# kostas1515/object_detectors

Measured on AMD Instinct MI355X. Metric: images/sec (fwd+bwd) YOLOv3 640px bs=32, higher is better.
Workload: dtype bf16; 1 GPU; YOLOv3 Darknet-53 training step (fwd+loss+bwd+SGD step), synthetic COCO 640px, per-GPU bs=32, 7 GT/img, random-init weights; global_batch=32, parallelism=dp1

## Files before the change

object_detectors_amd/csrc/wgrad_kernels.hip:

```cpp
#include "common.h"

#include <cstdlib>
#include <unordered_map>

#include "tune_record.h"

using namespace mi355;

typedef __attribute__((ext_vector_type(4))) short s16x4_t;
typedef __attribute__((ext_vector_type(4))) float f32x4_t;

struct FastDiv {
  unsigned mul, shift, d;
};

static FastDiv make_fastdiv(unsigned d) {
  FastDiv f;
  f.d = d;
  unsigned l = 0;
  while ((1ull << l) < d) ++l;
  f.shift = l;
  f.mul = (unsigned)(((1ull << 32) * ((1ull << l) - d)) / d + 1);
  return f;
}
__device__ __forceinline__ unsigned fdiv(unsigned n, const FastDiv f) {
  const unsigned t = __umulhi(f.mul, n);
  return (t + n) >> f.shift;
}

struct WgradParams {
  const bf16_t* x;
  const bf16_t* dy;
  float* dw;
  float* slab;
  const bf16_t* zero;
  int M, Ho, Wo, H, W, ldx, lddy, Cin, Cout, stride, pad, ks, T, NP;
  int co_tiles, np_tiles, splits, chunk;
  int step_q, step_r;
  FastDiv dWo, dHo, dCin;
  int ablate;
};

int g_wgrad_ablate = 0;
int g_wgrad_general = 0;
int g_conv_strict = 0;
int g_wgrad_force_dbg = 0;
int g_wgrad8_off = 0;

namespace {

#define WG_BKP 64
#define WG_TILE 128
#define WG_ROWB 256

__device__ __forceinline__ void glds16(const void* gsrc, void* lds_dst_uniform) {
  __builtin_amdgcn_global_load_lds((const __attribute__((address_space(1))) void*)gsrc,
                                   (__attribute__((address_space(3))) void*)lds_dst_uniform, 16, 0, 0);
}

typedef __attribute__((ext_vector_type(4))) int srd_t;
__device__ __forceinline__ srd_t make_srd(const void* base, unsigned num_records) {
  const unsigned long long a = (unsigned long long)base;
  srd_t r;
  r[0] = (int)(unsigned)a;
  r[1] = (int)((unsigned)(a >> 32) & 0xFFFFu);
  r[2] = (int)num_records;
  r[3] = 0x00020000;
  return r;
}
__device__ __forceinline__ void bufld16(srd_t rsrc, const void* lds_dst_uniform, int voffset, int soffset) {
  const unsigned lds = (unsigned)(unsigned long long)(__attribute__((address_space(3))) const void*)lds_dst_uniform;
  asm volatile("s_mov_b32 m0, %0\n\ts_nop 0\n\tbuffer_load_dwordx4 %1, %2, %3 offen lds" ::"s"(lds), "v"(voffset), "s"(rsrc), "s"(soffset) : "memory");
}
#define OOB_VOFF ((int)0x80000000)

__device__ __forceinline__ int rowf(int row) { return (row & 3) | (((row >> 3) & 1) << 2); }

__device__ __forceinline__ st16x4_t lds_tr(const char* p) {
  s16x4_t v = __builtin_amdgcn_ds_read_tr16_b64_v4i16((__attribute__((address_space(3))) s16x4_t*)p);
  return __builtin_bit_cast(st16x4_t, v);
}

template <int CI, int CJ, int GRP4>
__global__ __launch_bounds__(256, 2) void wgrad_kernel(const WgradParams p) {
  constexpr int STAGE = 2 * WG_BKP * WG_ROWB;
  extern __shared__ __attribute__((aligned(16))) char smem[];
  const int tid = threadIdx.x, lane = tid & 63;
  const int wid = __builtin_amdgcn_readfirstlane(tid >> 6);
  const int wr = wid & 1, wc = wid >> 1;

  int bid = blockIdx.x;
  {
    const int nblk = gridDim.x, q = nblk / 8, r = nblk % 8, xcd = bid % 8, loc = bid / 8;
    bid = (xcd < r ? xcd * (q + 1) : r * (q + 1) + (xcd - r) * q) + loc;
  }
  const int tiles = p.co_tiles * p.np_tiles;
  const int split = bid / tiles, tile = bid - split * tiles;
  const int ct = tile % p.co_tiles, nt = tile / p.co_tiles;
  const int co0 = ct * WG_TILE, np0 = nt * WG_TILE;
  const int mA = split * p.chunk, mB = min(p.M, mA + p.chunk);
  if (mA >= mB) return;

  const int lrow = lane >> 4, cpos = lane & 15;
  int x_off[2], x_tapdy[2], x_tapdx[2], dy_off[2];
  bool x_ok[2];
#pragma unroll
  for (int ph = 0; ph < 2; ++ph) {
    const int f = (lrow & 3) | (ph << 2);
    const int gchunk = (((cpos >> 1) ^ f) << 1) | (cpos & 1);
    dy_off[ph] = co0 + gchunk * 8;
    const int np = np0 + gchunk * 8;
    x_ok[ph] = np < p.NP;
    const int t = x_ok[ph] ? (int)fdiv((unsigned)np, p.dCin) : 0;
    const int ci = np - t * p.Cin;
    const int kh = t / p.ks, kw = t - kh * p.ks;
    x_tapdy[ph] = kh - p.pad;
    x_tapdx[ph] = kw - p.pad;
    x_off[ph] = ci;
  }
  const bool dy_ok0 = dy_off[0] < p.Cout, dy_ok1 = dy_off[1] < p.Cout;

  int r_n[4], r_ho[4], r_wo[4];
#pragma unroll
  for (int i = 0; i < 4; ++i) {
    if (GRP4) break;
    const unsigned um = (unsigned)(mA + (wid * 4 + i) * 4 + lrow);
    const unsigned q1 = fdiv(um, p.dWo);
    r_wo[i] = (int)(um - q1 * p.Wo);
    const unsigned n = fdiv(q1, p.dHo);
    r_ho[i] = (int)(q1 - n * p.Ho);
    r_n[i] = (int)n;
  }

  int g_hs[4], g_ws[4], g_sb[4], dyv[4], lc[2], ty[2], cx[2];
  srd_t rsrc_x;
  const int WoS = p.Wo * p.stride, HoS = p.Ho * p.stride;
  const int c_ws = p.step_r * p.stride, c_hs = p.step_q * p.stride;
  const int c_sb = (c_hs * p.W + c_ws) * p.ldx * 2;
  const int c_row = (p.stride * p.W - WoS) * p.ldx * 2;
  const int c_img = (p.H - HoS) * p.W * p.ldx * 2;
  const int c_piece = 4 * p.stride * p.ldx * 2;
  if constexpr (GRP4 != 0) {
#pragma unroll
    for (int i = 0; i < 4; ++i) {
      const unsigned um = (unsigned)(mA + (wid * 4 + i) * 4);
      const unsigned q1 = fdiv(um, p.dWo);
      const int wo = (int)(um - q1 * p.Wo);
      const unsigned n = fdiv(q1, p.dHo);
      const int ho = (int)(q1 - n * p.Ho);
      g_hs[i] = ho * p.stride;
      g_ws[i] = wo * p.stride;
      g_sb[i] = (((int)n * p.H + g_hs[i]) * p.W + g_ws[i]) * p.ldx * 2;
      const int ph = (i >> 1) & 1;
      dyv[i] = (ph ? dy_ok1 : dy_ok0) ? (((wid * 4 + i) * 4 + lrow) * p.lddy + dy_off[ph]) * 2 : OOB_VOFF;
    }
#pragma unroll
    for (int ph = 0; ph < 2; ++ph) {
      lc[ph] = (((x_tapdy[ph] + p.pad) * p.W + lrow * p.stride + x_tapdx[ph] + p.pad) * p.ldx + x_off[ph]) * 2;
      ty[ph] = x_ok[ph] ? x_tapdy[ph] : -(1 << 24);
      cx[ph] = lrow * p.stride + x_tapdx[ph];
    }
    rsrc_x = make_srd(p.x - (p.pad * p.W + p.pad) * p.ldx, 0x7FFFFFF0u);
  }
  auto stage_grp4 = [&](int m_base, int buf) {
    char* sd = smem + buf * STAGE;
    char* sx = sd + WG_BKP * WG_ROWB;
    const int rem = mB - m_base;
    const srd_t rsrc_dy = make_srd(p.dy + (long long)m_base * p.lddy, (unsigned)(rem * p.lddy * 2));
#pragma unroll
    for (int i = 0; i < 4; ++i) {
      const int instr = wid * 4 + i;
      const int ph = (i >> 1) & 1;
      if (!(p.ablate & 2) || m_base == mA) bufld16(rsrc_dy, sd + instr * 1024, dyv[i], 0);
      if (GRP4 == 3) {
        const int hs = g_hs[0], ws = g_ws[0] + i * 4 * p.stride;
        const bool ok = instr * 4 < rem && (unsigned)(hs + ty[ph]) < (unsigned)p.H && (unsigned)(ws + cx[ph]) < (unsigned)p.W;
        if (!(p.ablate & 1) || m_base == mA) bufld16(rsrc_x, sx + instr * 1024, ok ? lc[ph] : OOB_VOFF, g_sb[0] + i * c_piece);
        if (i < 3) continue;
      }
      const int ti = GRP4 == 3 ? 0 : i;
      const int hs = g_hs[ti], ws = g_ws[ti];
      if (GRP4 == 3) {
      } else if (GRP4 == 1 || (ws + 4 * p.stride <= WoS && instr * 4 + 4 <= rem)) {
        const bool ok = instr * 4 < rem && (unsigned)(hs + ty[ph]) < (unsigned)p.H && (unsigned)(ws + cx[ph]) < (unsigned)p.W;
        if (!(p.ablate & 1) || m_base == mA) bufld16(rsrc_x, sx + instr * 1024, ok ? lc[ph] : OOB_VOFF, g_sb[i]);
      } else {
        const bool last_row = hs + p.stride == HoS;
        const int hs1 = last_row ? 0 : hs + p.stride;
        const int ex1 = c_row + (last_row ? c_img : 0);
        const bool wr = ws + lrow * p.stride >= WoS;
        const int iy = (wr ? hs1 : hs) + ty[ph];
        const int ix = ws + cx[ph] - (wr ? WoS : 0);
        const bool ok = instr * 4 + lrow < rem && (unsigned)iy < (unsigned)p.H && (unsigned)ix < (unsigned)p.W;
        bufld16(rsrc_x, sx + instr * 1024, ok ? lc[ph] + (wr ? ex1 : 0) : OOB_VOFF, g_sb[i]);
      }
      g_ws[ti] += c_ws;
      g_hs[ti] += c_hs;
      g_sb[ti] += c_sb;
      if (g_ws[ti] >= WoS) {
        g_ws[ti] -= WoS;
        g_hs[ti] += p.stride;
        g_sb[ti] += c_row;
      }
      if (g_hs[ti] >= HoS) {
        g_hs[ti] -= HoS;
        g_sb[ti] += c_img;
      }
    }
  };

  auto stage_any = [&](int m_base, int buf) {
    char* sd = smem + buf * STAGE;
    char* sx = sd + WG_BKP * WG_ROWB;
#pragma unroll
    for (int i = 0; i < 4; ++i) {
      const int instr = wid * 4 + i;
      const int row = instr * 4 + lrow;
      const int ph = (row >> 3) & 1;
      const int m = m_base + row;
      const bool mv = m < mB;
      const bf16_t* sdy = (mv && (ph ? dy_ok1 : dy_ok0)) ? p.dy + (long long)m * p.lddy + (ph ? dy_off[1] : dy_off[0]) : p.zero;
      glds16(sdy, sd + instr * 1024);
      const int iy = r_ho[i] * p.stride + (ph ? x_tapdy[1] : x_tapdy[0]);
      const int ix = r_wo[i] * p.stride + (ph ? x_tapdx[1] : x_tapdx[0]);
      const bool ok = mv && (ph ? x_ok[1] : x_ok[0]) && iy >= 0 && iy < p.H && ix >= 0 && ix < p.W;
      const bf16_t* sxp = ok ? p.x + ((long long)(r_n[i] * p.H + iy) * p.W + ix) * p.ldx + (ph ? x_off[1] : x_off[0]) : p.zero;
      glds16(sxp, sx + instr * 1024);
      r_wo[i] += p.step_r;
      r_ho[i] += p.step_q;
      if (r_wo[i] >= p.Wo) {
        r_wo[i] -= p.Wo;
        r_ho[i] += 1;
      }
      while (r_ho[i] >= p.Ho) {
        r_ho[i] -= p.Ho;
        r_n[i] += 1;
      }
    }
  };

  auto stage = [&](int m_base, int buf) {
    if constexpr (GRP4 != 0)
      stage_grp4(m_base, buf);
    else
      stage_any(m_base, buf);
  };

  f32x4_t acc[CI][CJ];
#pragma unroll
  for (int i = 0; i < CI; ++i)
#pragma unroll
    for (int j = 0; j < CJ; ++j) acc[i][j] = {0.f, 0.f, 0.f, 0.f};

  const int ksteps = (mB - mA + WG_BKP - 1) / WG_BKP;
  stage(mA, 0);
  asm volatile("s_waitcnt vmcnt(0)" ::: "memory");
  __syncthreads();

  const int g = lane >> 4, q = (lane & 15) >> 2, pp = lane & 3;
  for (int s = 0; s < ksteps; ++s) {
    const int buf = s & 1;
    if (s + 1 < ksteps) stage(mA + (s + 1) * WG_BKP, buf ^ 1);
    const char* sd = smem + buf * STAGE;
    const char* sx = sd + WG_BKP * WG_ROWB;
#pragma unroll
    for (int ks = 0; ks < WG_BKP / 32; ++ks) {
      st16x8_t af[CI], bfr[CJ];
#pragma unroll
      for (int h = 0; h < 2; ++h) {
        const int row = ks * 32 + 8 * g + 4 * h + q;
        const int f = rowf(row);
#pragma unroll
        for (int i = 0; i < CI; ++i) {
          const int blk = wr * CI + i;
          const st16x4_t v = lds_tr(sd + row * WG_ROWB + ((blk ^ f) << 5) + pp * 8);
          af[i][4 * h + 0] = v[0];
          af[i][4 * h + 1] = v[1];
          af[i][4 * h + 2] = v[2];
          af[i][4 * h + 3] = v[3];
        }
#pragma unroll
        for (int j = 0; j < CJ; ++j) {
          const int blk = wc * CJ + j;
          const st16x4_t v = lds_tr(sx + row * WG_ROWB + ((blk ^ f) << 5) + pp * 8);
          bfr[j][4 * h + 0] = v[0];
          bfr[j][4 * h + 1] = v[1];
          bfr[j][4 * h + 2] = v[2];
          bfr[j][4 * h + 3] = v[3];
        }
      }
      if (!(p.ablate & 4)) {
#pragma unroll
        for (int i = 0; i < CI; ++i)
#pragma unroll
          for (int j = 0; j < CJ; ++j) acc[i][j] = MI355_MFMA_16x16x32(af[i], bfr[j], acc[i][j]);
      } else {
        acc[0][0][0] += (float)af[0][0] + (float)bfr[0][0];
      }
    }
    asm volatile("s_waitcnt vmcnt(0)" ::: "memory");
    __syncthreads();
  }

  const int fr = lane & 15, fq = lane >> 4;
  if (p.slab) {
    float* dst = p.slab + ((size_t)split * tiles + tile) * (WG_TILE * WG_TILE);
#pragma unroll
    for (int i = 0; i < CI; ++i)
#pragma unroll
      for (int r = 0; r < 4; ++r)
#pragma unroll
        for (int j = 0; j < CJ; ++j)
          dst[((wr * CI + i) * 16 + fq * 4 + r) * WG_TILE + (wc * CJ + j) * 16 + fr] = acc[i][j][r];
    return;
  }
#pragma unroll
  for (int i = 0; i < CI; ++i) {
#pragma unroll
    for (int r = 0; r < 4; ++r) {
      const int co = co0 + (wr * CI + i) * 16 + fq * 4 + r;
      if (co >= p.Cout) continue;
#pragma unroll
      for (int j = 0; j < CJ; ++j) {
        const int np = np0 + (wc * CJ + j) * 16 + fr;
        if (np < p.NP) p.dw[(long long)co * p.NP + np] += acc[i][j][r];
      }
    }
  }
}

constexpr int W8_HALF = WG_BKP * WG_ROWB;
constexpr int W8_STAGE = 4 * W8_HALF;
constexpr int W8_LDS = 2 * W8_STAGE;
constexpr int W8_TILE = 256;

template <int N>
__device__ __forceinline__ void w8_wait_vm() {
  asm volatile("s_waitcnt vmcnt(%0)" ::"n"(N) : "memory");
}
__device__ __forceinline__ void w8_bar() {
  asm volatile("" ::: "memory");
  __builtin_amdgcn_s_barrier();
  asm volatile("" ::: "memory");
}

template <bool STRADDLE>
__global__ __launch_bounds__(512, 2) void wgrad8_kernel(const WgradParams p) {
  extern __shared__ __attribute__((aligned(16))) char smem[];
  const int tid = threadIdx.x, lane = tid & 63;
  const int wid = __builtin_amdgcn_readfirstlane(tid >> 6);
  const int wm = wid >> 2, wn = wid & 3;

  int bid = blockIdx.x;
  {
    const int nblk = gridDim.x, q = nblk / 8, r = nblk % 8, xcd = bid % 8, loc = bid / 8;
    bid = (xcd < r ? xcd * (q + 1) : r * (q + 1) + (xcd - r) * q) + loc;
  }
  const int co_tiles8 = (p.Cout + W8_TILE - 1) / W8_TILE, np_tiles8 = (p.NP + W8_TILE - 1) / W8_TILE;
  const int tiles8 = co_tiles8 * np_tiles8;
  const int split = bid / tiles8, tile = bid - split * tiles8;
  const int CT = tile % co_tiles8, NT = tile / co_tiles8;
  const int co0 = CT * W8_TILE, np0 = NT * W8_TILE;
  const int mA = split * p.chunk, mB = min(p.M, mA + p.chunk);
  if (mA >= mB) return;
  const int mlen = mB - mA;

  const int lrow = lane >> 4, cpos = lane & 15;
  const int fst = lrow | ((wid & 1) << 2);
  const int gchunk = (((cpos >> 1) ^ fst) << 1) | (cpos & 1);
  int dyv[2][2], lc[2], ty[2], cx[2];
#pragma unroll
  for (int h = 0; h < 2; ++h) {
    const int co = co0 + (gchunk >> 2) * 64 + h * 32 + (gchunk & 3) * 8;
#pragma unroll
    for (int i = 0; i < 2; ++i) dyv[h][i] = co < p.Cout ? ((wid * 8 + i * 4 + lrow) * p.lddy + co) * 2 : OOB_VOFF;
    const int np = np0 + (gchunk >> 3) * 128 + h * 64 + (gchunk & 7) * 8;
    const bool x_ok = np < p.NP;
    const int t = x_ok ? (int)fdiv((unsigned)np, p.dCin) : 0;
    const int ci = np - t * p.Cin;
    const int kh = t / p.ks, kw = t - kh * p.ks;
    lc[h] = ((kh * p.W + lrow * p.stride + kw) * p.ldx + ci) * 2;
    ty[h] = x_ok ? kh - p.pad : -(1 << 24);
    cx[h] = lrow * p.stride + kw - p.pad;
  }
  const srd_t rsrc_x = make_srd(p.x - (p.pad * p.W + p.pad) * p.ldx, 0x7FFFFFF0u);
  const srd_t rsrc_dy = make_srd(p.dy + (long long)mA * p.lddy, (unsigned)((long long)mlen * p.lddy * 2));

  const int WoS = p.Wo * p.stride, HoS = p.Ho * p.stride;
  const int c_ws = p.step_r * p.stride, c_hs = p.step_q * p.stride;
  const int c_sb = (c_hs * p.W + c_ws) * p.ldx * 2;
  const int c_row = (p.stride * p.W - WoS) * p.ldx * 2;
  const int c_img = (p.H - HoS) * p.W * p.ldx * 2;
  int g_hs[2], g_ws[2], g_sb[2];
#pragma unroll
  for (int i = 0; i < 2; ++i) {
    const unsigned um = (unsigned)(mA + wid * 8 + i * 4);
    const unsigned q1 = fdiv(um, p.dWo);
    const int wo = (int)(um - q1 * p.Wo);
    const unsigned n = fdiv(q1, p.dHo);
    const int ho = (int)(q1 - n * p.Ho);
    g_hs[i] = ho * p.stride;
    g_ws[i] = wo * p.stride;
    g_sb[i] = (((int)n * p.H + g_hs[i]) * p.W + g_ws[i]) * p.ldx * 2;
  }
  struct Slot { int hs[2], ws[2], sb[2], dyoff, rem; };
  int pf = 0;
  auto next_slot = [&]() {
    Slot s;
    s.rem = mlen - pf;
    s.dyoff = pf * p.lddy * 2;
#pragma unroll
    for (int i = 0; i < 2; ++i) {
      s.hs[i] = g_hs[i];
      s.ws[i] = g_ws[i];
      s.sb[i] = g_sb[i];
      g_ws[i] += c_ws;
      g_hs[i] += c_hs;
      g_sb[i] += c_sb;
      if (g_ws[i] >= WoS) {
        g_ws[i] -= WoS;
        g_hs[i] += p.stride;
        g_sb[i] += c_row;
      }
      if (g_hs[i] >= HoS) {
        g_hs[i] -= HoS;
        g_sb[i] += c_img;
      }
    }
    pf += WG_BKP;
    return s;
  };
  auto issue_x = [&](const Slot& s, int h, int buf) {
    char* dst = smem + buf * W8_STAGE + h * W8_HALF + (2 * wid) * 1024;
#pragma unroll
    for (int i = 0; i < 2; ++i) {
      const int row0 = wid * 8 + i * 4;
      if (!STRADDLE || (s.ws[i] + 4 * p.stride <= WoS && row0 + 4 <= s.rem) || row0 >= s.rem) {
        const bool ok = row0 < s.rem && (unsigned)(s.hs[i] + ty[h]) < (unsigned)p.H && (unsigned)(s.ws[i] + cx[h]) < (unsigned)p.W;
        bufld16(rsrc_x, dst + i * 1024, ok ? lc[h] : OOB_VOFF, s.sb[i]);
      } else {
        const bool last_row = s.hs[i] + p.stride == HoS;
        const int hs1 = last_row ? 0 : s.hs[i] + p.stride;
        const int ex1 = c_row + (last_row ? c_img : 0);
        const bool wr = s.ws[i] + lrow * p.stride >= WoS;
        const int iy = (wr ? hs1 : s.hs[i]) + ty[h];
        const int ix = s.ws[i] + cx[h] - (wr ? WoS : 0);
        const bool ok = row0 + lrow < s.rem && (unsigned)iy < (unsigned)p.H && (unsigned)ix < (unsigned)p.W;
        bufld16(rsrc_x, dst + i * 1024, ok ? lc[h] + (wr ? ex1 : 0) : OOB_VOFF, s.sb[i]);
      }
    }
  };
  auto issue_d = [&](const Slot& s, int h, int buf) {
    char* dst = smem + buf * W8_STAGE + (2 + h) * W8_HALF + (2 * wid) * 1024;
#pragma unroll
    for (int i = 0; i < 2; ++i) bufld16(rsrc_dy, dst + i * 1024, s.rem > 0 ? dyv[h][i] + s.dyoff : OOB_VOFF, 0);
  };

  const int g = lane >> 4, q = (lane & 15) >> 2, pp = lane & 3;
  const int frd = q | ((g & 1) << 2);
  int xrd[4], drd[2];
#pragma unroll
  for (int jj = 0; jj < 4; ++jj) xrd[jj] = (8 * g + q) * WG_ROWB + pp * 8 + (((wm * 4 + jj) ^ frd) << 5);
#pragma unroll
  for (int ii = 0; ii < 2; ++ii) drd[ii] = 2 * W8_HALF + (8 * g + q) * WG_ROWB + pp * 8 + (((wn * 2 + ii) ^ frd) << 5);

  f32x4_t acc[4][8];
#pragma unroll
  for (int i = 0; i < 4; ++i)
#pragma unroll
    for (int j = 0; j < 8; ++j) acc[i][j] = {0.f, 0.f, 0.f, 0.f};

  const int ksteps = (mlen + WG_BKP - 1) / WG_BKP;
  Slot s1 = next_slot();
  issue_x(s1, 0, 0);
  issue_d(s1, 0, 0);
  issue_d(s1, 1, 0);
  issue_x(s1, 1, 0);
  s1 = next_slot();
  issue_x(s1, 0, 1);
  issue_d(s1, 0, 1);
  Slot s2 = next_slot();
  w8_wait_vm<6>();
  w8_bar();
  if (wm == 1) w8_bar();

  st16x8_t xf[2][4][2], df[2][2][2];
  auto rdd = [&](int h, int ks, bool nxt) {
#pragma unroll
    for (int ii = 0; ii < 2; ++ii)
#pragma unroll
      for (int hh = 0; hh < 2; ++hh) {
        const st16x4_t v = lds_tr(smem + (nxt ? (drd[ii] ^ W8_STAGE) : drd[ii]) + h * W8_HALF + (ks * 32 + hh * 4) * WG_ROWB);
        df[h][ii][ks][4 * hh + 0] = v[0];
        df[h][ii][ks][4 * hh + 1] = v[1];
        df[h][ii][ks][4 * hh + 2] = v[2];
        df[h][ii][ks][4 * hh + 3] = v[3];
      }
  };
  auto rdx = [&](int h, int ks, bool nxt) {
#pragma unroll
    for (int jj = 0; jj < 4; ++jj)
#pragma unroll
      for (int hh = 0; hh < 2; ++hh) {
        const st16x4_t v = lds_tr(smem + (nxt ? (xrd[jj] ^ W8_STAGE) : xrd[jj]) + h * W8_HALF + (ks * 32 + hh * 4) * WG_ROWB);
        xf[h][jj][ks][4 * hh + 0] = v[0];
        xf[h][jj][ks][4 * hh + 1] = v[1];
        xf[h][jj][ks][4 * hh + 2] = v[2];
        xf[h][jj][ks][4 * hh + 3] = v[3];
      }
  };
  auto mf = [&](int hd, int hx, int ks) {
#pragma unroll
    for (int ii = 0; ii < 2; ++ii)
#pragma unroll
      for (int jj = 0; jj < 4; ++jj)
        acc[hd * 2 + ii][hx * 4 + jj] = MI355_MFMA_16x16x32(df[hd][ii][ks], xf[hx][jj][ks], acc[hd * 2 + ii][hx * 4 + jj]);
  };
#define W8_INTERLEAVE(nm, nr)                                                      \
  do {                                                                            \
    _Pragma("unroll") for (int q_ = 0; q_ < ((nr) < (nm) ? (nr) : (nm)); ++q_) {   \
      __builtin_amdgcn_sched_group_barrier(0x008, 1, 0);                          \
      __builtin_amdgcn_sched_group_barrier(0x100, 1, 0);                          \
    }                                                                             \
    if constexpr ((nm) > (nr)) __builtin_amdgcn_sched_group_barrier(0x008, (nm) > (nr) ? (nm) - (nr) : 0, 0); \
    if constexpr ((nr) > (nm)) __builtin_amdgcn_sched_group_barrier(0x100, (nr) > (nm) ? (nr) - (nm) : 0, 0); \
  } while (0)

  rdd(0, 0, false);
  rdx(0, 0, false);
  rdx(0, 1, false);
  int buf = 0;
  for (int t = 0; t < ksteps; ++t) {
    issue_d(s1, 1, buf ^ 1);
    w8_wait_vm<8>();
    w8_bar();
    __builtin_amdgcn_sched_barrier(0);
    __builtin_amdgcn_s_setprio(1);
    rdd(0, 1, false);
    rdd(1, 0, false);
    mf(0, 0, 0);
    W8_INTERLEAVE(8, 8);
    rdd(1, 1, false);
    mf(0, 0, 1);
    W8_INTERLEAVE(8, 4);
    __builtin_amdgcn_s_setprio(0);
    __builtin_amdgcn_sched_barrier(0);
    w8_wait_vm<6>();
    w8_bar();
    issue_x(s1, 1, buf ^ 1);
    w8_wait_vm<8>();
    w8_bar();
    __builtin_amdgcn_sched_barrier(0);
    __builtin_amdgcn_s_setprio(1);
    rdx(1, 0, false);
    mf(1, 0, 0);
    W8_INTERLEAVE(8, 8);
    rdx(1, 1, false);
    mf(1, 0, 1);
    W8_INTERLEAVE(8, 8);
    __builtin_amdgcn_s_setprio(0);
    __builtin_amdgcn_sched_barrier(0);
    w8_wait_vm<6>();
    w8_bar();
    issue_x(s2, 0, buf);
    w8_wait_vm<8>();
    w8_bar();
    __builtin_amdgcn_sched_barrier(0);
    __builtin_amdgcn_s_setprio(1);
    mf(1, 1, 0);
    mf(1, 1, 1);
    __builtin_amdgcn_s_setprio(0);
    __builtin_amdgcn_sched_barrier(0);
    w8_wait_vm<6>();
    w8_bar();
    issue_d(s2, 0, buf);
    w8_wait_vm<8>();
    w8_bar();
    __builtin_amdgcn_sched_barrier(0);
    __builtin_amdgcn_s_setprio(1);
    rdx(0, 0, true);
    mf(0, 1, 0);
    W8_INTERLEAVE(8, 8);
    rdd(0, 0, true);
    rdx(0, 1, true);
    mf(0, 1, 1);
    W8_INTERLEAVE(8, 12);
    __builtin_amdgcn_s_setprio(0);
    __builtin_amdgcn_sched_barrier(0);
    w8_wait_vm<6>();
    w8_bar();
    s1 = s2;
    s2 = next_slot();
    buf ^= 1;
#pragma unroll
    for (int jj = 0; jj < 4; ++jj) xrd[jj] ^= W8_STAGE;
#pragma unroll
    for (int ii = 0; ii < 2; ++ii) drd[ii] ^= W8_STAGE;
  }
#undef W8_INTERLEAVE
  if (wm == 0) w8_bar();
  w8_wait_vm<0>();

  const int fr = lane & 15, fq = lane >> 4;
  const int nt128 = NT * 2 + wm;
// ... 138 lines not shown
        }
      }
    }
    for (; m < pixels; m += stride) {
      const uint4 u = *(const uint4*)(x + m * ld + gl * 8);
      const unsigned uu[4] = {u.x, u.y, u.z, u.w};
#pragma unroll
      for (int e = 0; e < 4; ++e) {
        a[2 * e] += s2f((bf16_t)(uu[e] & 0xFFFF));
        a[2 * e + 1] += s2f((bf16_t)(uu[e] >> 16));
      }
    }
  }
#pragma unroll
  for (int k = 0; k < 8; ++k) red[threadIdx.x * 8 + k] = a[k];
  __syncthreads();
  if (pl == 0) {
#pragma unroll
    for (int k = 0; k < 8; ++k) {
      float t = 0.f;
      for (int r = 0; r < npl; ++r) t += red[(r * groups + gl) * 8 + k];
      partial0[(size_t)blockIdx.x * groups_all * 8 + (size_t)(g0 + gl) * 8 + k] = t;
    }
  }
}
__global__ __launch_bounds__(256) void colsum_fold_kernel(const float* __restrict__ partial, int rows, int c8, int c, float* __restrict__ out) {
  __shared__ float red[8][32];
  const int cl = threadIdx.x & 31, part = threadIdx.x >> 5;
  const int ch = blockIdx.x * 32 + cl;
  float s0 = 0.f, s1 = 0.f;
  if (ch < c) {
    int r = part;
    for (; r + 8 < rows; r += 16) {
      s0 += partial[(size_t)r * c8 + ch];
      s1 += partial[(size_t)(r + 8) * c8 + ch];
    }
    if (r < rows) s0 += partial[(size_t)r * c8 + ch];
  }
  red[part][cl] = s0 + s1;
  __syncthreads();
  if (part == 0 && ch < c) {
    float t = 0.f;
#pragma unroll
    for (int q = 0; q < 8; ++q) t += red[q][cl];
    out[ch] += t;
  }
}

__global__ __launch_bounds__(256) void colsum8_kernel(const bf16_t* __restrict__ x, int ld, int c, long long pixels, float* __restrict__ out) {
  __shared__ float red[256 * 8];
  const int groups = (c + 7) >> 3;
  const int npl = 256 / groups;
  const int gl = threadIdx.x % groups, pl = threadIdx.x / groups;
  float a[8];
#pragma unroll
  for (int k = 0; k < 8; ++k) a[k] = 0.f;
  if (pl < npl) {
    const long long stride = (long long)gridDim.x * npl;
    long long m = (long long)blockIdx.x * npl + pl;
    for (; m + stride < pixels; m += 2 * stride) {
      const uint4 u = *(const uint4*)(x + m * ld + gl * 8), v = *(const uint4*)(x + (m + stride) * ld + gl * 8);
      const unsigned uu[4] = {u.x, u.y, u.z, u.w}, vv[4] = {v.x, v.y, v.z, v.w};
#pragma unroll
      for (int q = 0; q < 4; ++q) {
        a[2 * q] += s2f((bf16_t)(uu[q] & 0xFFFF)) + s2f((bf16_t)(vv[q] & 0xFFFF));
        a[2 * q + 1] += s2f((bf16_t)(uu[q] >> 16)) + s2f((bf16_t)(vv[q] >> 16));
      }
    }
    for (; m < pixels; m += stride) {
      const uint4 u = *(const uint4*)(x + m * ld + gl * 8);
      const unsigned uu[4] = {u.x, u.y, u.z, u.w};
#pragma unroll
      for (int q = 0; q < 4; ++q) {
        a[2 * q] += s2f((bf16_t)(uu[q] & 0xFFFF));
        a[2 * q + 1] += s2f((bf16_t)(uu[q] >> 16));
      }
    }
  }
#pragma unroll
  for (int k = 0; k < 8; ++k) red[threadIdx.x * 8 + k] = a[k];
  __syncthreads();
  if (pl == 0) {
#pragma unroll
    for (int k = 0; k < 8; ++k) {
      float t = 0.f;
      for (int r = 0; r < npl; ++r) t += red[(r * groups + gl) * 8 + k];
      if (gl * 8 + k < c) atomicAdd(out + gl * 8 + k, t);
    }
  }
}

int choose_splits(int tiles, int M, double out_bytes) {
  (void)out_bytes;
  int sp = max(1, min(1024, 512 / max(1, tiles)));
  sp = max(1, min(sp, M / 2048));
  while (sp > 1) {
    const int chunk = ((M + sp - 1) / sp + WG_BKP - 1) / WG_BKP * WG_BKP;
    if ((M + chunk - 1) / chunk == sp) break;
    --sp;
  }
  return sp;
}

TuneMap& g_wgrad_tuned = tune_table(TUNE_WGRAD);
int g_wgrad_force = 0;
constexpr int WG_FORM8 = 1 << 16;

unsigned long long wgrad_key(const mi355det_conv_shape* s) {
  unsigned long long k = (unsigned long long)(s->n * s->ho * s->wo);
  k = k * 4099 + s->cout;
  k = k * 4099 + s->cin;
  k = k * 17 + s->ksize * 4 + s->stride;
  k = k * 2 + MI355_F16;
  return k;
}

bool split_valid(int M, int sp) {
  const int chunk = ((M + sp - 1) / sp + WG_BKP - 1) / WG_BKP * WG_BKP;
  return (M + chunk - 1) / chunk == sp;
}

bf16_t* g_zero_page_w = nullptr;
int ensure_zero_page_w() {
  if (g_zero_page_w) return 0;
  void* p = nullptr;
  if (hipMalloc(&p, 4096) != hipSuccess || hipMemset(p, 0, 4096) != hipSuccess) return fail(MI355DET_ELAUNCH, "%s: zero page alloc failed", "wgrad");
  g_zero_page_w = (bf16_t*)p;
  return 0;
}

bool wgrad8_applicable(const mi355det_conv_shape* s) {
  const long long NP = (long long)s->ksize * s->ksize * s->cin;
  if (s->wo < 4 || WG_BKP / s->wo + 1 > s->ho || s->cout < 256 || NP < 256 || s->cin % 8 != 0) return false;
  return ((long long)s->n * s->h * s->w + (long long)s->pad * (s->w + 1)) * s->in_ld * 2 < 0x7FFFFFF0ll;
}

}

extern "C" {

size_t mi355det_conv_wgrad_workspace(const mi355det_conv_shape* s) {
  if (!s) return 0;
  const size_t tiles = (size_t)((s->cout + WG_TILE - 1) / WG_TILE) * (size_t)((s->ksize * s->ksize * s->cin + WG_TILE - 1) / WG_TILE);
  const size_t per_split = tiles * WG_TILE * WG_TILE * sizeof(float);
  size_t splits = 1024;
  while (splits > 3 && splits * per_split > ((size_t)128 << 20)) --splits;
  return splits * per_split;
}

int mi355det_conv_wgrad_autotune(const mi355det_conv_shape* s, const void* x, const void* dy, float* dw, void* workspace,
                                 size_t workspace_bytes, void* stream) {
  if (!s) return fail(MI355DET_EINVAL, "%s: null shape", "wgrad_autotune");
  if (tune_locked_has(TUNE_WGRAD, wgrad_key(s))) return g_wgrad_tuned[wgrad_key(s)];
  const int M = s->n * s->ho * s->wo;
  const size_t tiles = (size_t)((s->cout + WG_TILE - 1) / WG_TILE) * (size_t)((s->ksize * s->ksize * s->cin + WG_TILE - 1) / WG_TILE);
  const size_t per_split = tiles * WG_TILE * WG_TILE * sizeof(float);
  const int cands[] = {1, 2, 3, 4, 5, 6, 7, 8, 10, 12, 14, 16, 20, 24, 28, 32, 40, 48, 56, 64, 96, 128, 192, 256, 384, 512, 768, 1024};
  hipEvent_t e0, e1;
  if (hipEventCreate(&e0) != hipSuccess || hipEventCreate(&e1) != hipSuccess) return fail(MI355DET_ELAUNCH, "%s: event create failed", "wgrad_autotune");
  int best = -1;
  float best_ms = 1e30f;
  int tried[32], n_tried = 0;
  float tried_ms[32];
  for (int sp : cands) {
    if (sp > 1 && (sp * per_split > workspace_bytes || M / sp < 512 || (size_t)sp * tiles > 4096)) continue;
    if (!split_valid(M, sp)) continue;
    g_wgrad_force = sp;
    int e = mi355det_conv_wgrad(s, x, dy, dw, nullptr, workspace, workspace_bytes, stream);
    if (e) {
      g_wgrad_force = 0;
      (void)hipEventDestroy(e0);
      (void)hipEventDestroy(e1);
      return e;
    }
    float ms = 1e30f;
    for (int b = 0; b < 2; ++b) {
      (void)hipEventRecord(e0, S(stream));
      for (int r = 0; r < 3; ++r) (void)mi355det_conv_wgrad(s, x, dy, dw, nullptr, workspace, workspace_bytes, stream);
      (void)hipEventRecord(e1, S(stream));
      (void)hipEventSynchronize(e1);
      float t = 0.f;
      (void)hipEventElapsedTime(&t, e0, e1);
      if (t < ms) ms = t;
    }
    tried[n_tried] = sp;
    tried_ms[n_tried++] = ms;
    if (ms < best_ms) {
      best_ms = ms;
      best = sp;
    }
  }
  int best8 = -1;
  float best8_ms = 1e30f;
  if (wgrad8_applicable(s) && !g_wgrad8_off) {
    const int t8 = (int)(((s->cout + 255) / 256) * ((s->ksize * s->ksize * s->cin + 255) / 256));
    int c8[7] = {256 / t8, 512 / t8, 128 / t8, 768 / t8, 1, 2, 3};
    for (int a = 0; a < 7; ++a) {
      const int sp = c8[a];
      bool dup = sp < 1;
      for (int b = 0; b < a; ++b) dup = dup || c8[b] == sp;
      if (dup || (sp > 1 && (sp * per_split > workspace_bytes || M / sp < 512)) || !split_valid(M, sp)) continue;
      g_wgrad_force = sp | WG_FORM8;
      if (int e = mi355det_conv_wgrad(s, x, dy, dw, nullptr, workspace, workspace_bytes, stream)) {
        g_wgrad_force = 0;
        (void)hipEventDestroy(e0);
        (void)hipEventDestroy(e1);
        return e;
      }
      float ms = 1e30f;
      for (int b = 0; b < 2; ++b) {
        (void)hipEventRecord(e0, S(stream));
        for (int r = 0; r < 3; ++r) (void)mi355det_conv_wgrad(s, x, dy, dw, nullptr, workspace, workspace_bytes, stream);
        (void)hipEventRecord(e1, S(stream));
        (void)hipEventSynchronize(e1);
        float t = 0.f;
        (void)hipEventElapsedTime(&t, e0, e1);
        if (t < ms) ms = t;
      }
      if (ms < best8_ms) {
        best8_ms = ms;
        best8 = sp;
      }
    }
  }
  for (int i = 0; i < n_tried; ++i)
    if (tried_ms[i] <= best_ms * 1.04f) {
      best = tried[i];
      break;
    }
  if (best8 > 0 && best8_ms < best_ms * 0.97f) best = best8 | WG_FORM8;
  g_wgrad_force = 0;
  (void)hipEventDestroy(e0);
  (void)hipEventDestroy(e1);
  if (best > 0) {
    g_wgrad_tuned[wgrad_key(s)] = best;
    tune_mark_timed(TUNE_WGRAD, wgrad_key(s));
  }
  return best;
}

int mi355det_conv_wgrad(const mi355det_conv_shape* s, const void* x, const void* dy, float* dw, float* dbias, void* workspace,
                        size_t workspace_bytes, void* stream) {
  if (!s) return fail(MI355DET_EINVAL, "%s: null shape", "conv_wgrad");
  if (int e = ensure_zero_page_w()) return e;
  if (s->cin % 8 != 0) return fail(MI355DET_EINVAL, "%s: Cin must be a multiple of 8 (got %lld)", "conv_wgrad", s->cin);
  if (s->out_ld % 8 != 0 || s->in_ld % 8 != 0) return fail(MI355DET_EINVAL, "%s: pixel pitches must be multiples of 8", "conv_wgrad");
  WgradParams p{};
  p.x = (const bf16_t*)x;
  p.dy = (const bf16_t*)dy;
  p.dw = dw;
  p.zero = g_zero_page_w;
  p.M = s->n * s->ho * s->wo;
  p.Ho = s->ho; p.Wo = s->wo; p.H = s->h; p.W = s->w;
  p.ldx = s->in_ld; p.lddy = s->out_ld;
  p.Cin = s->cin; p.Cout = s->cout; p.stride = s->stride; p.pad = s->pad; p.ks = s->ksize;
  p.T = s->ksize * s->ksize;
  p.NP = p.T * p.Cin;
  p.co_tiles = (p.Cout + WG_TILE - 1) / WG_TILE;
  p.np_tiles = (p.NP + WG_TILE - 1) / WG_TILE;
  p.ablate = g_wgrad_ablate;
  const int tiles = p.co_tiles * p.np_tiles;
  int splits = choose_splits(tiles, p.M, 4.0 * p.Cout * (double)p.NP);
  bool form8 = false;
  {
    auto it = g_wgrad_tuned.find(wgrad_key(s));
    if (it != g_wgrad_tuned.end()) {
      splits = it->second & (WG_FORM8 - 1);
      form8 = (it->second & WG_FORM8) != 0;
    }
    const int force = g_wgrad_force > 0 ? g_wgrad_force : g_wgrad_force_dbg;
    if (g_conv_strict && g_wgrad_force <= 0 && g_wgrad_force_dbg > 0) {
      const int sp = g_wgrad_force_dbg & (WG_FORM8 - 1);
      const size_t need = (size_t)sp * tiles * WG_TILE * WG_TILE * sizeof(float);
      if (!split_valid(p.M, sp))
        return fail(MI355DET_EINVAL, "%s: forced split count %lld is not valid for %lld pixels (strict mode, debug key 9)", "conv_wgrad", sp, p.M);
      if (sp > 1 && (!workspace || need > workspace_bytes))
        return fail(MI355DET_EINVAL, "%s: forced split count %lld needs %lld workspace bytes (strict mode, debug key 9)", "conv_wgrad", sp, (long long)need);
    }
    if (force > 0 && split_valid(p.M, force & (WG_FORM8 - 1))) {
      splits = force & (WG_FORM8 - 1);
      form8 = (force & WG_FORM8) != 0;
    }
    if (splits < 1) splits = 1;
    if (g_wgrad_force <= 0 && (g_wgrad_force_dbg & WG_FORM8) && !(form8 && wgrad8_applicable(s)))
      return fail(MI355DET_EINVAL, "%s: the phase-staggered kernel was forced (debug key 7) for a shape or split count it does not take", "conv_wgrad");
    form8 = form8 && wgrad8_applicable(s);
    const size_t per_split = (size_t)tiles * WG_TILE * WG_TILE * sizeof(float);
    while (splits > 1 && (splits * per_split > workspace_bytes || !split_valid(p.M, splits))) --splits;
  }
  int chunk = (p.M + splits - 1) / splits;
  chunk = (chunk + WG_BKP - 1) / WG_BKP * WG_BKP;
  splits = (p.M + chunk - 1) / chunk;
  p.splits = splits;
  p.chunk = chunk;
  p.slab = nullptr;
  if (splits > 1) {
    const size_t need = (size_t)splits * tiles * WG_TILE * WG_TILE * sizeof(float);
    if (!workspace || workspace_bytes < need) return fail(MI355DET_EWORKSPACE, "%s: workspace too small (%lld bytes needed)", "conv_wgrad", (long long)need);
    if (p.NP % 4 != 0) return fail(MI355DET_EINVAL, "%s: k*k*Cin must be a multiple of 4", "conv_wgrad");
    p.slab = (float*)workspace;
  }
  p.step_q = WG_BKP / p.Wo;
  p.step_r = WG_BKP % p.Wo;
  p.dWo = make_fastdiv((unsigned)p.Wo);
  p.dHo = make_fastdiv((unsigned)p.Ho);
  p.dCin = make_fastdiv((unsigned)p.Cin);
  const int lds = 2 * 2 * WG_BKP * WG_ROWB;
  const int ci = p.Cout <= 32 ? 1 : (p.Cout <= 64 ? 2 : 4), cj = p.NP <= 32 ? 1 : (p.NP <= 64 ? 2 : 4);
  auto go = [&](auto kern) {
    (void)hipFuncSetAttribute((const void*)kern, hipFuncAttributeMaxDynamicSharedMemorySize, lds);
    hipLaunchKernelGGL(kern, dim3(tiles * splits), dim3(256), lds, S(stream), p);
  };
  const int grp4 = g_wgrad_general != 0 || p.Wo < 4 || WG_BKP / p.Wo + 1 > p.Ho ? 0 : (p.Wo % 16 == 0 ? 3 : (p.Wo % 4 == 0 ? 1 : 2));
  const bool fits =
                    ((long long)s->n * p.H * p.W + (long long)p.pad * (p.W + 1)) * p.ldx * 2 < 0x7FFFFFF0ll &&
                    (long long)chunk * p.lddy * 2 < 0x7FFFFFF0ll;
  if (form8 && !fits && g_conv_strict && g_wgrad_force <= 0 && (g_wgrad_force_dbg & WG_FORM8))
    return fail(MI355DET_EINVAL, "%s: the forced phase-staggered kernel does not fit the 31-bit offsets of this shape (strict mode, debug key 9)", "conv_wgrad");
  if (form8 && fits) {
    const int tiles8 = ((p.Cout + W8_TILE - 1) / W8_TILE) * ((p.NP + W8_TILE - 1) / W8_TILE);
    static DeviceOnce attr8;
    attr8.once([&] {
      (void)hipFuncSetAttribute((const void*)wgrad8_kernel<false>, hipFuncAttributeMaxDynamicSharedMemorySize, W8_LDS);
      (void)hipFuncSetAttribute((const void*)wgrad8_kernel<true>, hipFuncAttributeMaxDynamicSharedMemorySize, W8_LDS);
    });
    if (p.Wo % 4 == 0 && p.M % 4 == 0) hipLaunchKernelGGL(wgrad8_kernel<false>, dim3(tiles8 * splits), dim3(512), W8_LDS, S(stream), p);
    else hipLaunchKernelGGL(wgrad8_kernel<true>, dim3(tiles8 * splits), dim3(512), W8_LDS, S(stream), p);
  } else
#define WG_GO(a, b) (!fits || grp4 == 0 ? go(wgrad_kernel<a, b, 0>) : grp4 == 1 ? go(wgrad_kernel<a, b, 1>) : grp4 == 2 ? go(wgrad_kernel<a, b, 2>) : go(wgrad_kernel<a, b, 3>))
  switch (ci * 8 + cj) {
    case 1 * 8 + 1: WG_GO(1, 1); break;
    case 1 * 8 + 2: WG_GO(1, 2); break;
    case 1 * 8 + 4: WG_GO(1, 4); break;
    case 2 * 8 + 1: WG_GO(2, 1); break;
    case 2 * 8 + 2: WG_GO(2, 2); break;
    case 2 * 8 + 4: WG_GO(2, 4); break;
    case 4 * 8 + 1: WG_GO(4, 1); break;
    case 4 * 8 + 2: WG_GO(4, 2); break;
    default: WG_GO(4, 4); break;
  }
#undef WG_GO
  if (p.slab) {
    const long long total = (long long)p.Cout * (p.NP / 4);
    if (splits >= 8) {
      const int gx = (int)min((long long)4096, (total + 31) / 32);
      hipLaunchKernelGGL(wgrad_reduce8_kernel, dim3(gx), dim3(256), 0, S(stream), p.slab, dw, p.Cout, p.NP, p.co_tiles, p.np_tiles, splits);
    } else {
      const int gx = (int)min((long long)2048, (total + 255) / 256);
      hipLaunchKernelGGL(wgrad_reduce_kernel, dim3(gx, 1), dim3(256), 0, S(stream), p.slab, dw, p.Cout, p.NP, p.co_tiles, p.np_tiles, splits);
    }
  }
  if (dbias) {
    const int groups = (s->cout + 7) / 8;
    const bool vec = s->out_ld % 8 == 0 && groups * 8 <= s->out_ld && (((uintptr_t)dy) & 15) == 0;
    const int npl = 256 / (groups < 256 ? groups : 256);
    const int gp = (int)max(1ll, min((long long)512, ((long long)p.M + (long long)npl * 8 - 1) / ((long long)npl * 8)));
    if (vec && gp > 1 && workspace && workspace_bytes >= (size_t)gp * groups * 8 * sizeof(float)) {
      hipLaunchKernelGGL(colsum8p_kernel, dim3(gp, (groups + 255) / 256), dim3(256), 0, S(stream), (const bf16_t*)dy, s->out_ld, s->cout, (long long)p.M, (float*)workspace);
      hipLaunchKernelGGL(colsum_fold_kernel, dim3((s->cout + 31) / 32), dim3(256), 0, S(stream), (const float*)workspace, gp, groups * 8, s->cout, dbias);
    } else if (vec && groups <= 256) {
      const int gx = (int)max(1ll, min((long long)128, ((long long)p.M + (long long)npl * 16 - 1) / ((long long)npl * 16)));
      hipLaunchKernelGGL(colsum8_kernel, dim3(gx), dim3(256), 0, S(stream), (const bf16_t*)dy, s->out_ld, s->cout, (long long)p.M, dbias);
    } else {
      const int gy = (int)min((long long)256, ((long long)p.M + 255) / 256);
      hipLaunchKernelGGL(colsum_kernel, dim3((p.Cout + 63) / 64, gy), dim3(256), 0, S(stream), (const bf16_t*)dy, s->out_ld, s->cout, (long long)p.M, dbias);
    }
  }
  return check_launch("conv_wgrad");
}

}
```

Baseline: 1157 images/s.

## Replace double-buffered wgrad staging with a 4-deep ring of 32-row stages

The generic wgrad kernel now stages 32 M-rows per step into a four-slot LDS ring instead of double-buffering 64-row stages. Each step waits only for the oldest in-flight stage with a partial vmcnt and needs a single barrier, so global-to-LDS loads stay three stages ahead of the MFMA work. The aim is to hide more load latency and drop the full vmcnt(0) drain every iteration. The trade-off is more barriers per unit of work, since each step is half as big, plus a delicate hand-counted vmcnt scheme and reworked address bookkeeping.

```diff
diff --git a/object_detectors_amd/csrc/wgrad_kernels.hip b/object_detectors_amd/csrc/wgrad_kernels.hip
--- a/object_detectors_amd/csrc/wgrad_kernels.hip
+++ b/object_detectors_amd/csrc/wgrad_kernels.hip
@@ -37,6 +37,7 @@
   int M, Ho, Wo, H, W, ldx, lddy, Cin, Cout, stride, pad, ks, T, NP;
   int co_tiles, np_tiles, splits, chunk;
   int step_q, step_r;
+  int hstep_q, hstep_r;
   FastDiv dWo, dHo, dCin;
   int ablate;
 };
@@ -50,12 +51,15 @@
 namespace {
 
 #define WG_BKP 64
+#define WG_STG 32
+#define WG_RING 4
+#define WG_LPS 4
 #define WG_TILE 128
 #define WG_ROWB 256
 
-__device__ __forceinline__ void glds16(const void* gsrc, void* lds_dst_uniform) {
-  __builtin_amdgcn_global_load_lds((const __attribute__((address_space(1))) void*)gsrc,
-                                   (__attribute__((address_space(3))) void*)lds_dst_uniform, 16, 0, 0);
+__device__ __forceinline__ void glds16a(const void* gsrc, const void* lds_dst_uniform) {
+  const unsigned lds = (unsigned)(unsigned long long)(__attribute__((address_space(3))) const void*)lds_dst_uniform;
+  asm volatile("s_mov_b32 m0, %0\n\ts_nop 0\n\tglobal_load_lds_dwordx4 %1, off" ::"s"(lds), "v"(gsrc) : "memory");
 }
 
 typedef __attribute__((ext_vector_type(4))) int srd_t;
@@ -81,9 +85,20 @@
   return __builtin_bit_cast(st16x4_t, v);
 }
 
+template <int N>
+__device__ __forceinline__ void wg_wait_stage() {
+  asm volatile("s_waitcnt vmcnt(%0) lgkmcnt(0)" ::"n"(N) : "memory");
+}
+__device__ __forceinline__ void wg_bar() {
+  asm volatile("" ::: "memory");
+  __builtin_amdgcn_s_barrier();
+  asm volatile("" ::: "memory");
+}
+
 template <int CI, int CJ, int GRP4>
 __global__ __launch_bounds__(256, 2) void wgrad_kernel(const WgradParams p) {
-  constexpr int STAGE = 2 * WG_BKP * WG_ROWB;
+  constexpr int HALF = WG_STG * WG_ROWB;
+  constexpr int STAGE = 2 * HALF;
   extern __shared__ __attribute__((aligned(16))) char smem[];
   const int tid = threadIdx.x, lane = tid & 63;
   const int wid = __builtin_amdgcn_readfirstlane(tid >> 6);
@@ -102,29 +117,21 @@
   if (mA >= mB) return;
 
   const int lrow = lane >> 4, cpos = lane & 15;
-  int x_off[2], x_tapdy[2], x_tapdx[2], dy_off[2];
-  bool x_ok[2];
-#pragma unroll
-  for (int ph = 0; ph < 2; ++ph) {
-    const int f = (lrow & 3) | (ph << 2);
-    const int gchunk = (((cpos >> 1) ^ f) << 1) | (cpos & 1);
-    dy_off[ph] = co0 + gchunk * 8;
-    const int np = np0 + gchunk * 8;
-    x_ok[ph] = np < p.NP;
-    const int t = x_ok[ph] ? (int)fdiv((unsigned)np, p.dCin) : 0;
-    const int ci = np - t * p.Cin;
-    const int kh = t / p.ks, kw = t - kh * p.ks;
-    x_tapdy[ph] = kh - p.pad;
-    x_tapdx[ph] = kw - p.pad;
-    x_off[ph] = ci;
-  }
-  const bool dy_ok0 = dy_off[0] < p.Cout, dy_ok1 = dy_off[1] < p.Cout;
-
-  int r_n[4], r_ho[4], r_wo[4];
-#pragma unroll
-  for (int i = 0; i < 4; ++i) {
+  const int gchunk = (((cpos >> 1) ^ (lrow | ((wid & 1) << 2))) << 1) | (cpos & 1);
+  const int dy_off = co0 + gchunk * 8;
+  const bool dy_ok = dy_off < p.Cout;
+  const int x_np = np0 + gchunk * 8;
+  const bool x_ok = x_np < p.NP;
+  const int x_t = x_ok ? (int)fdiv((unsigned)x_np, p.dCin) : 0;
+  const int x_off = x_np - x_t * p.Cin;
+  const int x_kh = x_t / p.ks;
+  const int x_tapdy = x_kh - p.pad, x_tapdx = x_t - x_kh * p.ks - p.pad;
+
+  int r_n[2], r_ho[2], r_wo[2];
+#pragma unroll
+  for (int i = 0; i < 2; ++i) {
     if (GRP4) break;
-    const unsigned um = (unsigned)(mA + (wid * 4 + i) * 4 + lrow);
+    const unsigned um = (unsigned)(mA + (wid * 2 + i) * 4 + lrow);
     const unsigned q1 = fdiv(um, p.dWo);
     r_wo[i] = (int)(um - q1 * p.Wo);
     const unsigned n = fdiv(q1, p.dHo);
@@ -132,18 +139,18 @@
     r_n[i] = (int)n;
   }
 
-  int g_hs[4], g_ws[4], g_sb[4], dyv[4], lc[2], ty[2], cx[2];
+  int g_hs[2], g_ws[2], g_sb[2], dyv[2], lc = 0, ty = 0, cx = 0;
   srd_t rsrc_x;
   const int WoS = p.Wo * p.stride, HoS = p.Ho * p.stride;
-  const int c_ws = p.step_r * p.stride, c_hs = p.step_q * p.stride;
+  const int c_ws = p.hstep_r * p.stride, c_hs = p.hstep_q * p.stride;
   const int c_sb = (c_hs * p.W + c_ws) * p.ldx * 2;
   const int c_row = (p.stride * p.W - WoS) * p.ldx * 2;
   const int c_img = (p.H - HoS) * p.W * p.ldx * 2;
   const int c_piece = 4 * p.stride * p.ldx * 2;
   if constexpr (GRP4 != 0) {
 #pragma unroll
-    for (int i = 0; i < 4; ++i) {
-      const unsigned um = (unsigned)(mA + (wid * 4 + i) * 4);
+    for (int i = 0; i < 2; ++i) {
+      const unsigned um = (unsigned)(mA + (wid * 2 + i) * 4);
       const unsigned q1 = fdiv(um, p.dWo);
       const int wo = (int)(um - q1 * p.Wo);
       const unsigned n = fdiv(q1, p.dHo);
@@ -151,48 +158,44 @@
       g_hs[i] = ho * p.stride;
       g_ws[i] = wo * p.stride;
       g_sb[i] = (((int)n * p.H + g_hs[i]) * p.W + g_ws[i]) * p.ldx * 2;
-      const int ph = (i >> 1) & 1;
-      dyv[i] = (ph ? dy_ok1 : dy_ok0) ? (((wid * 4 + i) * 4 + lrow) * p.lddy + dy_off[ph]) * 2 : OOB_VOFF;
-    }
-#pragma unroll
-    for (int ph = 0; ph < 2; ++ph) {
-      lc[ph] = (((x_tapdy[ph] + p.pad) * p.W + lrow * p.stride + x_tapdx[ph] + p.pad) * p.ldx + x_off[ph]) * 2;
-      ty[ph] = x_ok[ph] ? x_tapdy[ph] : -(1 << 24);
-      cx[ph] = lrow * p.stride + x_tapdx[ph];
-    }
+      dyv[i] = dy_ok ? (((wid * 2 + i) * 4 + lrow) * p.lddy + dy_off) * 2 : OOB_VOFF;
+    }
+    lc = (((x_tapdy + p.pad) * p.W + lrow * p.stride + x_tapdx + p.pad) * p.ldx + x_off) * 2;
+    ty = x_ok ? x_tapdy : -(1 << 24);
+    cx = lrow * p.stride + x_tapdx;
     rsrc_x = make_srd(p.x - (p.pad * p.W + p.pad) * p.ldx, 0x7FFFFFF0u);
   }
+  const int m_ring = mA + WG_RING * WG_STG;
   auto stage_grp4 = [&](int m_base, int buf) {
     char* sd = smem + buf * STAGE;
-    char* sx = sd + WG_BKP * WG_ROWB;
+    char* sx = sd + HALF;
     const int rem = mB - m_base;
     const srd_t rsrc_dy = make_srd(p.dy + (long long)m_base * p.lddy, (unsigned)(rem * p.lddy * 2));
 #pragma unroll
-    for (int i = 0; i < 4; ++i) {
-      const int instr = wid * 4 + i;
-      const int ph = (i >> 1) & 1;
-      if (!(p.ablate & 2) || m_base == mA) bufld16(rsrc_dy, sd + instr * 1024, dyv[i], 0);
+    for (int i = 0; i < 2; ++i) {
+      const int instr = wid * 2 + i;
+      if (!(p.ablate & 2) || m_base < m_ring) bufld16(rsrc_dy, sd + instr * 1024, dyv[i], 0);
       if (GRP4 == 3) {
         const int hs = g_hs[0], ws = g_ws[0] + i * 4 * p.stride;
-        const bool ok = instr * 4 < rem && (unsigned)(hs + ty[ph]) < (unsigned)p.H && (unsigned)(ws + cx[ph]) < (unsigned)p.W;
-        if (!(p.ablate & 1) || m_base == mA) bufld16(rsrc_x, sx + instr * 1024, ok ? lc[ph] : OOB_VOFF, g_sb[0] + i * c_piece);
-        if (i < 3) continue;
+        const bool ok = instr * 4 < rem && (unsigned)(hs + ty) < (unsigned)p.H && (unsigned)(ws + cx) < (unsigned)p.W;
+        if (!(p.ablate & 1) || m_base < m_ring) bufld16(rsrc_x, sx + instr * 1024, ok ? lc : OOB_VOFF, g_sb[0] + i * c_piece);
+        if (i < 1) continue;
       }
       const int ti = GRP4 == 3 ? 0 : i;
       const int hs = g_hs[ti], ws = g_ws[ti];
       if (GRP4 == 3) {
       } else if (GRP4 == 1 || (ws + 4 * p.stride <= WoS && instr * 4 + 4 <= rem)) {
-        const bool ok = instr * 4 < rem && (unsigned)(hs + ty[ph]) < (unsigned)p.H && (unsigned)(ws + cx[ph]) < (unsigned)p.W;
-        if (!(p.ablate & 1) || m_base == mA) bufld16(rsrc_x, sx + instr * 1024, ok ? lc[ph] : OOB_VOFF, g_sb[i]);
+        const bool ok = instr * 4 < rem && (unsigned)(hs + ty) < (unsigned)p.H && (unsigned)(ws + cx) < (unsigned)p.W;
+        if (!(p.ablate & 1) || m_base < m_ring) bufld16(rsrc_x, sx + instr * 1024, ok ? lc : OOB_VOFF, g_sb[i]);
       } else {
         const bool last_row = hs + p.stride == HoS;
         const int hs1 = last_row ? 0 : hs + p.stride;
         const int ex1 = c_row + (last_row ? c_img : 0);
-        const bool wr = ws + lrow * p.stride >= WoS;
-        const int iy = (wr ? hs1 : hs) + ty[ph];
-        const int ix = ws + cx[ph] - (wr ? WoS : 0);
+        const bool wrp = ws + lrow * p.stride >= WoS;
+        const int iy = (wrp ? hs1 : hs) + ty;
+        const int ix = ws + cx - (wrp ? WoS : 0);
         const bool ok = instr * 4 + lrow < rem && (unsigned)iy < (unsigned)p.H && (unsigned)ix < (unsigned)p.W;
-        bufld16(rsrc_x, sx + instr * 1024, ok ? lc[ph] + (wr ? ex1 : 0) : OOB_VOFF, g_sb[i]);
+        bufld16(rsrc_x, sx + instr * 1024, ok ? lc + (wrp ? ex1 : 0) : OOB_VOFF, g_sb[i]);
       }
       g_ws[ti] += c_ws;
       g_hs[ti] += c_hs;
@@ -211,23 +214,21 @@
 
   auto stage_any = [&](int m_base, int buf) {
     char* sd = smem + buf * STAGE;
-    char* sx = sd + WG_BKP * WG_ROWB;
-#pragma unroll
-    for (int i = 0; i < 4; ++i) {
-      const int instr = wid * 4 + i;
-      const int row = instr * 4 + lrow;
-      const int ph = (row >> 3) & 1;
-      const int m = m_base + row;
+    char* sx = sd + HALF;
+#pragma unroll
+    for (int i = 0; i < 2; ++i) {
+      const int instr = wid * 2 + i;
+      const int m = m_base + instr * 4 + lrow;
       const bool mv = m < mB;
-      const bf16_t* sdy = (mv && (ph ? dy_ok1 : dy_ok0)) ? p.dy + (long long)m * p.lddy + (ph ? dy_off[1] : dy_off[0]) : p.zero;
-      glds16(sdy, sd + instr * 1024);
-      const int iy = r_ho[i] * p.stride + (ph ? x_tapdy[1] : x_tapdy[0]);
-      const int ix = r_wo[i] * p.stride + (ph ? x_tapdx[1] : x_tapdx[0]);
-      const bool ok = mv && (ph ? x_ok[1] : x_ok[0]) && iy >= 0 && iy < p.H && ix >= 0 && ix < p.W;
-      const bf16_t* sxp = ok ? p.x + ((long long)(r_n[i] * p.H + iy) * p.W + ix) * p.ldx + (ph ? x_off[1] : x_off[0]) : p.zero;
-      glds16(sxp, sx + instr * 1024);
-      r_wo[i] += p.step_r;
-      r_ho[i] += p.step_q;
+      const bf16_t* sdy = (mv && dy_ok) ? p.dy + (long long)m * p.lddy + dy_off : p.zero;
+      glds16a(sdy, sd + instr * 1024);
+      const int iy = r_ho[i] * p.stride + x_tapdy;
+      const int ix = r_wo[i] * p.stride + x_tapdx;
+      const bool ok = mv && x_ok && iy >= 0 && iy < p.H && ix >= 0 && ix < p.W;
+      const bf16_t* sxp = ok ? p.x + ((long long)(r_n[i] * p.H + iy) * p.W + ix) * p.ldx + x_off : p.zero;
+      glds16a(sxp, sx + instr * 1024);
+      r_wo[i] += p.hstep_r;
+      r_ho[i] += p.hstep_q;
       if (r_wo[i] >= p.Wo) {
         r_wo[i] -= p.Wo;
         r_ho[i] += 1;
@@ -252,54 +253,55 @@
 #pragma unroll
     for (int j = 0; j < CJ; ++j) acc[i][j] = {0.f, 0.f, 0.f, 0.f};
 
-  const int ksteps = (mB - mA + WG_BKP - 1) / WG_BKP;
-  stage(mA, 0);
-  asm volatile("s_waitcnt vmcnt(0)" ::: "memory");
-  __syncthreads();
+  const int nst = (mB - mA + WG_STG - 1) / WG_STG;
+#pragma unroll
+  for (int d = 0; d < WG_RING - 1; ++d)
+    if (d < nst) stage(mA + d * WG_STG, d);
 
   const int g = lane >> 4, q = (lane & 15) >> 2, pp = lane & 3;
-  for (int s = 0; s < ksteps; ++s) {
-    const int buf = s & 1;
-    if (s + 1 < ksteps) stage(mA + (s + 1) * WG_BKP, buf ^ 1);
-    const char* sd = smem + buf * STAGE;
-    const char* sx = sd + WG_BKP * WG_ROWB;
-#pragma unroll
-    for (int ks = 0; ks < WG_BKP / 32; ++ks) {
-      st16x8_t af[CI], bfr[CJ];
-#pragma unroll
-      for (int h = 0; h < 2; ++h) {
-        const int row = ks * 32 + 8 * g + 4 * h + q;
-        const int f = rowf(row);
-#pragma unroll
-        for (int i = 0; i < CI; ++i) {
-          const int blk = wr * CI + i;
-          const st16x4_t v = lds_tr(sd + row * WG_ROWB + ((blk ^ f) << 5) + pp * 8);
-          af[i][4 * h + 0] = v[0];
-          af[i][4 * h + 1] = v[1];
-          af[i][4 * h + 2] = v[2];
-          af[i][4 * h + 3] = v[3];
-        }
-#pragma unroll
-        for (int j = 0; j < CJ; ++j) {
-          const int blk = wc * CJ + j;
-          const st16x4_t v = lds_tr(sx + row * WG_ROWB + ((blk ^ f) << 5) + pp * 8);
-          bfr[j][4 * h + 0] = v[0];
-          bfr[j][4 * h + 1] = v[1];
-          bfr[j][4 * h + 2] = v[2];
-          bfr[j][4 * h + 3] = v[3];
-        }
-      }
-      if (!(p.ablate & 4)) {
-#pragma unroll
-        for (int i = 0; i < CI; ++i)
-#pragma unroll
-          for (int j = 0; j < CJ; ++j) acc[i][j] = MI355_MFMA_16x16x32(af[i], bfr[j], acc[i][j]);
-      } else {
-        acc[0][0][0] += (float)af[0][0] + (float)bfr[0][0];
-      }
-    }
-    asm volatile("s_waitcnt vmcnt(0)" ::: "memory");
-    __syncthreads();
+  for (int s = 0; s < nst; ++s) {
+    if (s + WG_RING - 2 < nst)
+      wg_wait_stage<(WG_RING - 2) * WG_LPS>();
+    else if (s + 1 < nst)
+      wg_wait_stage<WG_LPS>();
+    else
+      wg_wait_stage<0>();
+    wg_bar();
+    if (s + WG_RING - 1 < nst) stage(mA + (s + WG_RING - 1) * WG_STG, (s + WG_RING - 1) % WG_RING);
+    const char* sd = smem + (s % WG_RING) * STAGE;
+    const char* sx = sd + HALF;
+    st16x8_t af[CI], bfr[CJ];
+#pragma unroll
+    for (int h = 0; h < 2; ++h) {
+      const int row = 8 * g + 4 * h + q;
+      const int f = rowf(row);
+#pragma unroll
+      for (int i = 0; i < CI; ++i) {
+        const int blk = wr * CI + i;
+        const st16x4_t v = lds_tr(sd + row * WG_ROWB + ((blk ^ f) << 5) + pp * 8);
+        af[i][4 * h + 0] = v[0];
+        af[i][4 * h + 1] = v[1];
+        af[i][4 * h + 2] = v[2];
+        af[i][4 * h + 3] = v[3];
+      }
+#pragma unroll
+      for (int j = 0; j < CJ; ++j) {
+        const int blk = wc * CJ + j;
+        const st16x4_t v = lds_tr(sx + row * WG_ROWB + ((blk ^ f) << 5) + pp * 8);
+        bfr[j][4 * h + 0] = v[0];
+        bfr[j][4 * h + 1] = v[1];
+        bfr[j][4 * h + 2] = v[2];
+        bfr[j][4 * h + 3] = v[3];
+      }
+    }
+    if (!(p.ablate & 4)) {
+#pragma unroll
+      for (int i = 0; i < CI; ++i)
+#pragma unroll
+        for (int j = 0; j < CJ; ++j) acc[i][j] = MI355_MFMA_16x16x32(af[i], bfr[j], acc[i][j]);
+    } else {
+      acc[0][0][0] += (float)af[0][0] + (float)bfr[0][0];
+    }
   }
 
   const int fr = lane & 15, fq = lane >> 4;
@@ -1044,10 +1046,12 @@
   }
   p.step_q = WG_BKP / p.Wo;
   p.step_r = WG_BKP % p.Wo;
+  p.hstep_q = WG_STG / p.Wo;
+  p.hstep_r = WG_STG % p.Wo;
   p.dWo = make_fastdiv((unsigned)p.Wo);
   p.dHo = make_fastdiv((unsigned)p.Ho);
   p.dCin = make_fastdiv((unsigned)p.Cin);
-  const int lds = 2 * 2 * WG_BKP * WG_ROWB;
+  const int lds = WG_RING * 2 * WG_STG * WG_ROWB;
   const int ci = p.Cout <= 32 ? 1 : (p.Cout <= 64 ? 2 : 4), cj = p.NP <= 32 ? 1 : (p.NP <= 64 ? 2 : 4);
   auto go = [&](auto kern) {
     (void)hipFuncSetAttribute((const void*)kern, hipFuncAttributeMaxDynamicSharedMemorySize, lds);
```

Result: slower. 1132 images/s (-2.2%).
